# 3DAnimals/3DAnimals

Measured on AMD Instinct MI355X. Metric: train images/sec fwd+bwd @256x256 b16, higher is better.
Workload: dtype f32

## Files before the change

3danimals_amd/_lib.py:

```python
from __future__ import annotations

import ctypes
import os

import torch

_HERE = os.path.dirname(os.path.abspath(__file__))
LIB_PATH = os.environ.get("A3D_LIB") or os.path.join(_HERE, "lib", "liba3d_hip.so")

_c_int, _c_float, _c_size_t, _p = ctypes.c_int, ctypes.c_float, ctypes.c_size_t, ctypes.c_void_p

SIGNATURES = {
    "a3d_version": (_c_int, []),
    "a3d_last_error": (ctypes.c_char_p, []),
    "a3d_bw_probe_fill": (_c_int, [_p, ctypes.c_int64, _p]),
    "a3d_bw_probe_read": (_c_int, [_p, ctypes.c_int64, _p, _p]),
    "a3d_dmtet_scratch_bytes": (_c_size_t, [_c_int, _c_int]),
    "a3d_dmtet_count": (_c_int, [_p, _p, _p, _c_int, _c_int, _p, _p, _p, _c_int, _c_int, _p, _p, _c_int, _p, _c_int, _p]),
    "a3d_dmtet_count_ordered": (_c_int, [_p, _c_int, _c_int, _c_int, _p, _p, _p, _p, _c_int, _p, _c_int, _p]),
    "a3d_dmtet_word_group_slots": (_c_int, []),
    "a3d_dmtet_word_group_bits": (_c_int, []),
    "a3d_dmtet_block_items": (_c_int, []),
    "a3d_dmtet_vertex_scratch_bytes": (_c_size_t, [_c_int]),
    "a3d_dmtet_gather_rows": (_c_int, [_p, _p, ctypes.c_int64, ctypes.c_int64, _c_int, _p, _p]),
# ... 95 lines not shown
    _fields_ = [("size", ctypes.c_uint32), ("lists_stride", ctypes.c_int32), ("prev_rast", _p), ("cover_scratch", _p), ("aa_screen", _p),
                ("aa_count", _p), ("topo_off", _p), ("topo_adj", _p), ("topo_opp", _p), ("normals_v_a", _p), ("normals_v_b", _p),
                ("normals_off", _p), ("normals_adj", _p), ("normals_acc_a", _p), ("normals_a", _p), ("normals_acc_b", _p), ("normals_b", _p),
                ("normals_B_a", ctypes.c_int32), ("normals_B_b", ctypes.c_int32), ("bins", _p), ("bin_cap", ctypes.c_int32), ("bins_clean", ctypes.c_int32),
                ("defer_resolve", ctypes.c_int32), ("reserved", ctypes.c_int32)]


class AaRide(ctypes.Structure):

    _fields_ = [("size", ctypes.c_uint32), ("clip_batch", ctypes.c_int32), ("rast", _p), ("screen", _p), ("tri", _p), ("opp", _p), ("off", _p),
                ("adj", _p), ("V", ctypes.c_int32), ("F", ctypes.c_int32), ("lists_stride", ctypes.c_int32), ("reserved", ctypes.c_int32)]


class CaBuffer(ctypes.Structure):

    _fields_ = [("size", ctypes.c_uint32), ("C", ctypes.c_int32), ("vals", _p), ("bg", _p), ("out", _p), ("g_out", _p), ("g_vals", _p),
                ("bg_batch", ctypes.c_int32), ("reserved", ctypes.c_int32), ("bg_channels", ctypes.c_int32), ("g_stride", ctypes.c_int32),
                ("g_channels", ctypes.c_int32), ("out_channels", ctypes.c_int32), ("vals_rows", ctypes.c_int64)]


class CaShade(ctypes.Structure):

    _fields_ = [("size", ctypes.c_uint32), ("kd_stride", ctypes.c_int32), ("gb", _p), ("par", _p), ("kd", _p), ("clear", _p),
                ("n_clear", ctypes.c_int32), ("two_sided", ctypes.c_int32), ("params", _p), ("shaded_out", _p)]


class ShadeParams(ctypes.Structure):

    _fields_ = [("size", ctypes.c_uint32), ("rot_row_stride", ctypes.c_int32), ("rot", _p), ("view", _p), ("light", _p),
                ("rot_image_stride", ctypes.c_int64), ("view_image_stride", ctypes.c_int64), ("light_image_stride", ctypes.c_int64)]


class EstimateBonesArgs(ctypes.Structure):

    _fields_ = [("size", ctypes.c_uint32), ("N", ctypes.c_int32), ("pos", _p), ("bones", _p), ("nearest", _p), ("ok", _p), ("V", ctypes.c_int32),
                ("n_body", ctypes.c_int32), ("n_leg", ctypes.c_int32), ("body_mode_y_plus", ctypes.c_int32), ("use_y_threshold", ctypes.c_int32),
                ("y_threshold", ctypes.c_float), ("attach", ctypes.c_int32 * 4), ("blend", ctypes.c_float * 17), ("ramp", ctypes.c_float * 9), ("workspace", _p)]


class GbAux(ctypes.Structure):

    _fields_ = [("size", ctypes.c_uint32), ("reserved", ctypes.c_int32), ("tex_out", _p), ("img_out", _p), ("rows", ctypes.c_int64),
                ("pad_to", ctypes.c_int64)]


class DmtetEmitOpts(ctypes.Structure):

    _fields_ = [("size", ctypes.c_uint32), ("Nv", ctypes.c_int32), ("vertex_scratch", _p), ("surf_idx", _p), ("g_sdf_to_clear", _p), ("tri32", _p),
                ("topo_count", _p), ("topo_adj", _p), ("device_counts", _p), ("n_surf", ctypes.c_int32), ("topo_stride", ctypes.c_int32),
                ("use_block_lists", ctypes.c_int32), ("n_edge_blocks_listed", ctypes.c_int32), ("n_tet_blocks_listed", ctypes.c_int32),
                ("surf_bucket", ctypes.c_int32), ("surf_pts", _p)]


class TexDesc(ctypes.Structure):

    _fields_ = [("size", ctypes.c_uint32), ("C", ctypes.c_int32), ("tex_batch", ctypes.c_int32), ("filter", ctypes.c_int32), ("boundary", ctypes.c_int32),
                ("levels", ctypes.c_int32), ("height", ctypes.c_int32 * 16), ("width", ctypes.c_int32 * 16), ("level", _p * 16), ("grad", _p * 16)]


class EnvDesc(ctypes.Structure):

    _fields_ = [("size", ctypes.c_uint32), ("N", ctypes.c_int32), ("roughness", ctypes.c_float), ("costheta_cutoff", ctypes.c_float), ("src", _p),
                ("dst", _p), ("bounds", _p), ("area", _p)]


class BsdfDesc(ctypes.Structure):

    _fields_ = [("size", ctypes.c_uint32), ("op", ctypes.c_int32), ("variant", ctypes.c_int32), ("min_roughness", ctypes.c_float),
                ("ndim", ctypes.c_int32), ("reserved", ctypes.c_int32), ("shape", ctypes.c_int64 * 4), ("seg", ctypes.c_int64), ("in", _p * 6),
                ("stride", ctypes.c_int64 * 24), ("cstride", ctypes.c_int64 * 6), ("out", _p), ("scratch", _p), ("g_out", _p),
                ("g_mode", ctypes.c_int32 * 6), ("seg_div", ctypes.c_int64 * 6), ("g_in", _p * 6), ("g_final", _p * 6)]


BSDF_SIGNATURES = {
    "a3d_bsdf_rows": (ctypes.c_int64, [_p]),
    "a3d_bsdf_fwd": (_c_int, [_p, _p]),
    "a3d_bsdf_bwd": (_c_int, [_p, _p]),
    "a3d_image_loss_fwd": (_c_int, [_p, _p]),
    "a3d_image_loss_bwd": (_c_int, [_p, _p]),
}
BSDF_TILE = 1024
BSDF_MAX_DIMS = 4

ABI_VERSION = 404
_lib = None


class A3DError(RuntimeError):
    pass


def lib():
    global _lib
    if _lib is None:
        if not os.path.exists(LIB_PATH):
            raise A3DError(
                f"{LIB_PATH} is missing: build it with `python 3danimals_amd/csrc/build.py` "
                "(or __graft_entry__.build()).  There is no CPU fallback for the HIP hot path."
            )
        handle = ctypes.CDLL(LIB_PATH)
        for name, (res, args) in list(SIGNATURES.items()) + list(BSDF_SIGNATURES.items()):
            fn = getattr(handle, name)
            fn.restype, fn.argtypes = res, args
        if handle.a3d_version() != ABI_VERSION:
            raise A3DError(f"{LIB_PATH} has ABI version {handle.a3d_version()}, this package binds version {ABI_VERSION}: rebuild it "
                           "with `python 3danimals_amd/csrc/build.py`")
        _lib = handle
    return _lib


class KernelTimer:

    active = None

    def __init__(self):
        self.records = {}

    def __enter__(self):
        KernelTimer.active = self
        return self

    def __exit__(self, *exc):
        KernelTimer.active = None
        return False

    def summary(self):
        torch.cuda.synchronize()
        out = {}
        for name, pairs in self.records.items():
            ms = [a.elapsed_time(b) for a, b in pairs]
            out[name] = (len(ms), sum(ms) / max(len(ms), 1))
        return out


GUARD = int(os.environ.get("A3D_GUARD", "0") or 0)
GUARD_BYTES = 256
_GUARD_BYTE = 0xA5
_guard_live = []
guard_stats = dict(checks=0, buffers_checked=0, allocations=0)


def set_guard(level):
    global GUARD
    import importlib

    prev, GUARD = GUARD, int(level)
    ops = importlib.import_module(__package__ + ".ops")
    ops.torch = GuardedTorch(torch) if GUARD else torch
    if not GUARD:
        _guard_live.clear()
    return prev


def guarded_empty(shape, dtype, device, zero=False, site=""):
    dtype = dtype or torch.get_default_dtype()
    shape = tuple(int(v) for v in shape)
    n = 1
    for v in shape:
        n *= v
    item = torch.empty((), dtype=dtype).element_size()
    nbytes = n * item
    pad = (-nbytes) % 16
    base = torch.empty(GUARD_BYTES + nbytes + pad + GUARD_BYTES, dtype=torch.uint8, device=device)
    base[:GUARD_BYTES] = _GUARD_BYTE
    base[GUARD_BYTES + nbytes:] = _GUARD_BYTE
    t = base[GUARD_BYTES:GUARD_BYTES + nbytes].view(dtype).view(shape)
    if zero:
        t.zero_()
    elif GUARD >= 2 and n:
        if dtype.is_floating_point:
            t.fill_(float("nan"))
        elif dtype == torch.bool:
            t.fill_(True)
        elif item == 1:
            t.fill_(0x7F)
        else:
            t.fill_(0x7F7F7F7F if item >= 4 else 0x7F7F)
    _guard_live.append((base.untyped_storage(), nbytes, f"{dtype} {list(shape)} allocated at {site}"))
    guard_stats["allocations"] += 1
    return t


class GuardedTorch:

# ... 208 lines not shown
```

3danimals_amd/csrc/build.py:

```python
import os
import subprocess
import sys
from concurrent.futures import ThreadPoolExecutor

HERE = os.path.dirname(os.path.abspath(__file__))
PKG = os.path.dirname(HERE)
LIB_DIR = os.path.join(PKG, "lib")
LIB = os.path.join(LIB_DIR, "liba3d_hip.so")
OBJ_DIR = os.path.join(HERE, "build")

SOURCES = {
    "common.hip": [],
    "dmtet.hip": ["-ffp-contract=off"],
    "skin.hip": [],
    "bones.hip": [],
    "normals.hip": ["-ffp-contract=off"],
    "raster.hip": ["-ffp-contract=off"],
    "cover.hip": [],
    "shade.hip": ["-ffp-contract=off"],
    "interp.hip": [],
    "gbuffer.hip": [],
    "segsum.hip": [],
    "losses.hip": [],
    "embed.hip": ["-ffp-contract=off"],
    "gemm.hip": [],
    "antialias.hip": ["-ffp-contract=off"],
    "topology.hip": [],
    "xfm.hip": ["-ffp-contract=off"],
    "texture.hip": ["-ffp-contract=off"],
    "envlight.hip": ["-ffp-contract=off"],
    "bsdf.hip": ["-ffp-contract=off"],
}
COMMON = ["--offload-arch=gfx950", "-O3", "-std=c++17", "-fPIC", "-fhip-fp32-correctly-rounded-divide-sqrt", "-Wall",
          "-Wno-unused-function"]


def _hipcc():
    for c in (os.environ.get("HIPCC"), "/opt/rocm/bin/hipcc", "hipcc"):
        if c and (os.path.isabs(c) and os.path.exists(c) or not os.path.isabs(c)):
            return c
    raise RuntimeError("hipcc not found")


def _stale(target, deps):
    if not os.path.exists(target):
        return True
    t = os.path.getmtime(target)
    return any(os.path.getmtime(d) > t for d in deps)


def build(force=False, verbose=True, profile=False, exp=False):
    assert not (profile and exp)
    lib = os.path.join(LIB_DIR, "liba3d_hip_prof.so") if profile else (os.path.join(LIB_DIR, "liba3d_hip_exp.so") if exp else LIB)
    obj_dir = os.path.join(OBJ_DIR, "prof") if profile else (os.path.join(OBJ_DIR, "exp") if exp else OBJ_DIR)
    os.makedirs(LIB_DIR, exist_ok=True)
    os.makedirs(obj_dir, exist_ok=True)
    hipcc = _hipcc()
    headers = sorted(os.path.join(HERE, f) for f in os.listdir(HERE) if f.endswith(".h")) + [os.path.join(os.path.dirname(PKG), "include", h) for h in ("a3d.h", "a3d_bsdf.h")] + [os.path.abspath(__file__)]
    jobs = []
    objs = []
    for src, extra in SOURCES.items():
        s = os.path.join(HERE, src)
        o = os.path.join(obj_dir, src.replace(".hip", ".o"))
        objs.append(o)
        if force or _stale(o, [s] + headers):
            jobs.append([hipcc, "-x", "hip", "-c", s, "-o", o] + COMMON + extra + (["-DA3D_PROFILE"] if profile else []) + (["-DA3D_EXPERIMENT"] if exp else []))

    def run(cmd):
        if verbose:
            print(" ".join(cmd), flush=True)
        subprocess.check_call(cmd)

    with ThreadPoolExecutor(max_workers=min(8, max(1, len(jobs)))) as ex:
        list(ex.map(run, jobs))
    if force or jobs or _stale(lib, objs):
        run([hipcc, "--offload-arch=gfx950", "-shared", "-fPIC", "-o", lib] + objs)
    return lib


if __name__ == "__main__":
    print(build(force="--force" in sys.argv, profile="--profile" in sys.argv, exp="--exp" in sys.argv))
```

3danimals_amd/csrc/gemm.hip:

```cpp
#include "a3d_common.h"

namespace {

typedef float f32x16 __attribute__((ext_vector_type(16)));
typedef float f32x4 __attribute__((ext_vector_type(4)));

constexpr int GM_N = 256, GM_BK = 32, GM_APAD = GM_BK + 1;

template <int WM, int WN, int BN, int OCC, bool MASK>
__global__ __launch_bounds__(64 * WM * WN, OCC) void gm_nn_kernel(const float* __restrict__ A, const float* __restrict__ B,
                                                                  const float* __restrict__ X, int M, int K, float* __restrict__ C) {
    constexpr int BM = 32 * WM, NT = 64 * WM * WN, TN = BN / WN / 32;
    constexpr int A_F4 = BM * GM_BK / 4 / NT;
    constexpr int B_F4 = GM_BK * BN / 4 / NT;
    static_assert(A_F4 >= 1 && B_F4 >= 1 && BM * GM_BK / 4 % NT == 0 && GM_BK * BN / 4 % NT == 0, "tile / thread count mismatch");
    constexpr int A_ROWS_PER_PASS = NT / 8;
    constexpr int B_ROWS_PER_PASS = NT / (BN / 4);
    __shared__ float As[BM * GM_APAD];
    __shared__ float Bs[GM_BK * BN];
    const int tid = threadIdx.x, lane = tid & 63, wave = tid >> 6, wm = wave / WN, wn = wave - wm * WN;
    const long long m0 = (long long)blockIdx.x * BM;
    const int n0 = blockIdx.y * BN;

    f32x16 acc[TN];
#pragma unroll
    for (int j = 0; j < TN; ++j)
#pragma unroll
        for (int r = 0; r < 16; ++r) acc[j][r] = 0.f;

    static_assert(!MASK || TN == 4, "the masked path keeps the signs of its 64 outputs per lane in one 64-bit word");
    unsigned long long xmask = 0ull;
    const int col0 = n0 + wn * (BN / WN) + (lane & 31);
    const long long mrow = m0 + 32 * wm + 4 * (lane >> 5);
    const float* x_lane = MASK ? X + col0 : nullptr;
    const int a_row = tid >> 3, a_kq = tid & 7, b_row = tid / (BN / 4), b_nq = tid - b_row * (BN / 4);
    const float* a_src = A + (m0 + a_row) * K + 4 * a_kq;
    const float* b_src = B + (long long)b_row * GM_N + n0 + 4 * b_nq;
    f32x4 ra[A_F4], rb[B_F4];
    const f32x4 zero4 = {0.f, 0.f, 0.f, 0.f};
#pragma unroll
    for (int i = 0; i < A_F4; ++i)
        ra[i] = m0 + a_row + A_ROWS_PER_PASS * i < M ? *reinterpret_cast<const f32x4*>(a_src + (long long)A_ROWS_PER_PASS * i * K) : zero4;
#pragma unroll
    for (int i = 0; i < B_F4; ++i) rb[i] = *reinterpret_cast<const f32x4*>(b_src + (long long)B_ROWS_PER_PASS * i * GM_N);

    for (int k0 = 0; k0 < K; k0 += GM_BK) {
        __syncthreads();
#pragma unroll
        for (int i = 0; i < A_F4; ++i) {
            float* d = As + (a_row + A_ROWS_PER_PASS * i) * GM_APAD + 4 * a_kq;
            d[0] = ra[i].x; d[1] = ra[i].y; d[2] = ra[i].z; d[3] = ra[i].w;
        }
#pragma unroll
        for (int i = 0; i < B_F4; ++i) *reinterpret_cast<f32x4*>(Bs + (b_row + B_ROWS_PER_PASS * i) * BN + 4 * b_nq) = rb[i];
        __syncthreads();
        {
            const int kn = k0 + GM_BK < K ? k0 + GM_BK : 0;
            const float* ap = a_src + kn;
            const float* bp = b_src + (long long)kn * GM_N;
#pragma unroll
            for (int i = 0; i < A_F4; ++i)
                ra[i] = m0 + a_row + A_ROWS_PER_PASS * i < M ? *reinterpret_cast<const f32x4*>(ap + (long long)A_ROWS_PER_PASS * i * K) : zero4;
#pragma unroll
            for (int i = 0; i < B_F4; ++i) rb[i] = *reinterpret_cast<const f32x4*>(bp + (long long)B_ROWS_PER_PASS * i * GM_N);
        }
        float xv[MASK ? 8 : 1];
        if (MASK) {
            const int c = (k0 / GM_BK) & 7;
            const float* xb = x_lane + 32 * (c >> 1);
            const long long r0 = mrow + 16 * (c & 1);
#pragma unroll
            for (int dq = 0; dq < 2; ++dq)
#pragma unroll
                for (int sx = 0; sx < 4; ++sx) {
                    const long long rr = r0 + 8 * dq + sx;
                    xv[4 * dq + sx] = xb[(rr < M ? rr : M - 1) * GM_N];
                }
        }
        const float* a_base = As + (32 * wm + (lane & 31)) * GM_APAD + (lane >> 5);
        const float* b_base = Bs + (lane >> 5) * BN + wn * (BN / WN) + (lane & 31);
        float av_n = a_base[0], bv_n[TN];
#pragma unroll
        for (int j = 0; j < TN; ++j) bv_n[j] = b_base[32 * j];
// ... 48 lines not shown
    const int n0 = half * G3_BN;
#pragma unroll
    for (int i = 0; i < 8; ++i) {
        const int f = tid + 1024 * i, k = f >> 5, q = f & 31;
        *reinterpret_cast<f32x4*>(Bs + k * G3_BN + 4 * q) = *reinterpret_cast<const f32x4*>(B + (long long)k * GM_N + n0 + 4 * q);
    }
    __syncthreads();

    const int row = lane & 31, kh = lane >> 5;
    const int n_tiles = (M + 31) >> 5;
    const int stride = nb * G3_WAVES;
    const float* b_lane = Bs + 4 * kh * G3_BN + row;
    for (int t = (wave >> 2) * (nb * 4) + bid * 4 + (wave & 3); t < n_tiles; t += stride) {
        const long long m0 = 32ll * t;
        const long long mr = m0 + row < M ? m0 + row : M - 1;
        const float* a_lane = A + mr * K + 4 * kh;
        f32x16 acc[TN];
#pragma unroll
        for (int j = 0; j < TN; ++j)
#pragma unroll
            for (int r = 0; r < 16; ++r) acc[j][r] = 0.f;
        const long long mrow = m0 + 4 * kh;
        const float* x_wave = MASK ? X + n0 + 4 * row : nullptr;

        f32x4 an[4];
#pragma unroll
        for (int i = 0; i < 4; ++i) an[i] = *reinterpret_cast<const f32x4*>(a_lane + 8 * i);
#pragma unroll 1
        for (int c = 0; c < 8; ++c) {
            f32x4 av[4];
#pragma unroll
            for (int i = 0; i < 4; ++i) av[i] = an[i];
            {
                const int cn = c + 1 < 8 ? c + 1 : 0;
#pragma unroll
                for (int i = 0; i < 4; ++i) an[i] = *reinterpret_cast<const f32x4*>(a_lane + 32 * cn + 8 * i);
            }
            f32x4 xw[MASK ? 2 : 1];
            if (MASK) {
#pragma unroll
                for (int q = 0; q < 2; ++q) {
                    long long rr = m0 + 2 * (2 * c + q) + kh;
                    rr = rr < M ? rr : M - 1;
                    xw[q] = *reinterpret_cast<const f32x4*>(x_wave + rr * GM_N);
                }
            }
            const float* bc = b_lane + (32 * c) * G3_BN;
#pragma unroll
            for (int g = 0; g < 4; ++g)
#pragma unroll
                for (int u = 0; u < 4; ++u) {
                    const float* bp = bc + (8 * g + u) * G3_BN;
#pragma unroll
                    for (int j = 0; j < TN; ++j) acc[j] = __builtin_amdgcn_mfma_f32_32x32x2f32(av[g][u], bp[32 * j], acc[j], 0, 0, 0);
                }
            if (MASK) {
#pragma unroll
                for (int q = 0; q < 2; ++q)
#pragma unroll
                    for (int k4 = 0; k4 < 4; ++k4) {
                        const unsigned long long bal = __ballot(xw[q][k4] > 0.f);
                        if (lane == 0) sign_w[(2 * c + q) * 4 + k4] = bal;
                    }
            }
        }
        if (MASK) __builtin_amdgcn_fence(__ATOMIC_ACQ_REL, "wavefront");
#pragma unroll
        for (int r = 0; r < 16; ++r) {
            const long long m = mrow + (r & 3) + 8 * (r >> 2);
            unsigned long long wv = 0ull;
            if (MASK) wv = sign_w[(2 * kh + ((r & 3) >> 1) + 4 * (r >> 2)) * 4 + (row & 3)] >> ((r & 1) * 32 + (row >> 2));
            if (m < M) {
#pragma unroll
                for (int j = 0; j < TN; ++j) {
                    float v = acc[j][r];
                    if (MASK) v = (wv >> (8 * j)) & 1ull ? v : 0.f;
                    C[m * GM_N + n0 + 32 * j + row] = v;
                }
            }
        }
    }
}

}

extern "C" int a3d_gemm_nn_relumask(const float* A, const float* B, const float* X, int64_t M, int N, int K, float* C, a3d_stream_t stream) {
    A3D_CHECK_ARG(M >= 0 && N == GM_N && K > 0 && K % GM_BK == 0 && M < 0x7fffffffll);
    A3D_CHECK_ARG(X == nullptr || K >= 256);
    if (M == 0) return A3D_OK;
    A3D_CHECK_ARG(A && B && C);
    hipStream_t s = (hipStream_t)stream;
#ifdef A3D_EXPERIMENT
    static const int variant = getenv("A3D_GEMM_VARIANT") ? atoi(getenv("A3D_GEMM_VARIANT")) : 3;
#else
    const int variant = 3;
#endif
    const dim3 block256(256);
    if (variant == 3 && K == 256) {
        static int n_cu_of[64] = {0};
        int dev = 0;
        A3D_HIP(hipGetDevice(&dev));
        A3D_CHECK_ARG(dev >= 0 && dev < 64);
        if (!n_cu_of[dev]) {
            int n = 0;
            A3D_HIP(hipDeviceGetAttribute(&n, hipDeviceAttributeMultiprocessorCount, dev));
            A3D_HIP(hipFuncSetAttribute(reinterpret_cast<const void*>(gm_nn3_kernel<true>), hipFuncAttributeMaxDynamicSharedMemorySize, (256 * G3_BN * 4 + 16 * 64 * 8)));
            A3D_HIP(hipFuncSetAttribute(reinterpret_cast<const void*>(gm_nn3_kernel<false>), hipFuncAttributeMaxDynamicSharedMemorySize, (256 * G3_BN * 4 + 16 * 64 * 8)));
            n_cu_of[dev] = n;
        }
        const int n_cu = n_cu_of[dev];
        const dim3 grid(n_cu & ~1), block(64 * G3_WAVES);
        if (X) hipLaunchKernelGGL(gm_nn3_kernel<true>, grid, block, (256 * G3_BN * 4 + 16 * 64 * 8), s, A, B, X, (int)M, C);
        else hipLaunchKernelGGL(gm_nn3_kernel<false>, grid, block, (256 * G3_BN * 4 + 16 * 64 * 8), s, A, B, X, (int)M, C);
        A3D_LAUNCH_CHECK();
        return A3D_OK;
    }
    if (variant == 1) {
        const dim3 grid(a3d_div_up(M, 64), 1);
        if (X) hipLaunchKernelGGL((gm_nn_kernel<2, 2, 256, 3, true>), grid, block256, 0, s, A, B, X, (int)M, K, C);
        else hipLaunchKernelGGL((gm_nn_kernel<2, 2, 256, 3, false>), grid, block256, 0, s, A, B, X, (int)M, K, C);
    } else {
        const dim3 grid(a3d_div_up(M, 128), 2);
        if (X) hipLaunchKernelGGL((gm_nn_kernel<4, 1, 128, 3, true>), grid, block256, 0, s, A, B, X, (int)M, K, C);
        else hipLaunchKernelGGL((gm_nn_kernel<4, 1, 128, 4, false>), grid, block256, 0, s, A, B, X, (int)M, K, C);
    }
    A3D_LAUNCH_CHECK();
    return A3D_OK;
}
```

3danimals_amd/ops.py:

```python
from __future__ import annotations

import ctypes
import math
import os
from collections import OrderedDict

import torch

from . import _lib
from ._lib import call, f32c, f32h, ptr, require_device, stream


class _IdentityCache:

    def __init__(self, maxsize=8):
        self.maxsize = maxsize
        self.data = OrderedDict()

    @staticmethod
    def key(t):
        return (t.data_ptr(), tuple(t.shape), t.dtype, t._version)

    def get(self, t, make):
        k = self.key(t)
# ... 1582 lines not shown
    def backward(ctx, g_loss, _g_both=None):
        shaded, dino, image_gt, dino_gt, mask_gt, dt0, dt1, valid, both = ctx.saved_tensors
        B, H, W = shaded.shape[:3]
        D = 0 if dino is None else dino.shape[3]
        if g_loss is None:
            return (None,) * 8
        g_shaded = torch.empty_like(shaded)
        ds = dino.stride(2) if D else 0
        g_dino = torch.empty((B, H, W, ds), dtype=torch.float32, device=shaded.device)[..., :D] if D else None
        call("a3d_recon_losses_bwd", ptr(f32h(g_loss)), ptr(shaded), ptr(dino), D, ds, ds, ptr(image_gt), ptr(dino_gt), ptr(mask_gt), ptr(dt0), ptr(dt1),
             dt0.stride(0), ptr(valid), B, H, W, ptr(both), ptr(g_shaded), ptr(g_dino), stream())
        return g_shaded, g_dino, None, None, None, None, None, None


def reconstruction_losses(shaded_nchw, dino_nchw, image_gt, dino_gt, mask_gt, mask_dt, mask_valid, return_mask=False):
    shaded = shaded_nchw.permute(0, 2, 3, 1)
    shaded = shaded if shaded.is_contiguous() else shaded.contiguous()
    dino = None
    if dino_nchw is not None:
        dino = dino_nchw.permute(0, 2, 3, 1)
        H, W, S = dino.shape[1], dino.shape[2], dino.stride(2)
        if not (dino.dtype == torch.float32 and dino.stride(3) == 1 and S >= dino.shape[3] and dino.stride(1) == W * S and dino.stride(0) == H * W * S):
            dino = dino.contiguous()
    loss, both = _ReconLosses.apply(shaded, dino, image_gt, dino_gt, mask_gt, mask_dt[:, 0], mask_dt[:, 1], mask_valid)
    return (loss, both) if return_mask else loss


class _FlowLoss(torch.autograd.Function):
    @staticmethod
    def forward(ctx, flow, flow_gt, both, B, F):
        require_device(flow, flow_gt, both, what="flow_loss")
        N, H, W = flow.shape[:3]
        assert N == B * F and F >= 2 and flow.shape[3] == 2 and flow.stride(3) == 1 and flow.stride(1) == W * flow.stride(2) \
            and flow.stride(0) == H * flow.stride(1), "flow must be the renderer's NHWC buffer (channel slice allowed)"
        flow_gt = f32c(flow_gt)
        assert flow_gt.shape == (B, F - 1, 2, H, W) and both.numel() == N * H * W
        loss = torch.empty((B, F - 1), dtype=torch.float32, device=flow.device)
        scale = torch.empty_like(loss)
        scratch = torch.empty(_lib.lib().a3d_flow_loss_scratch_bytes(B, F, H, W), dtype=torch.uint8, device=flow.device)
        call("a3d_flow_loss_fwd", ptr(flow), flow.stride(2), ptr(flow_gt), ptr(both), B, F, H, W, ptr(scratch), ptr(loss), ptr(scale), stream())
        ctx.save_for_backward(flow, flow_gt, both, scale)
        ctx.dims = (B, F, H, W)
        return loss

    @staticmethod
    def backward(ctx, g_loss):
        flow, flow_gt, both, scale = ctx.saved_tensors
        B, F, H, W = ctx.dims
        g_flow = torch.empty((B * F, H, W, 2), dtype=torch.float32, device=flow.device)
        call("a3d_flow_loss_bwd", ptr(f32h(g_loss)), ptr(scale), ptr(flow), flow.stride(2), ptr(flow_gt), ptr(both), B, F, H, W, ptr(g_flow), stream())
        return g_flow, None, None, None, None


def flow_loss(flow_nchw, flow_gt, both, batch, num_frames):
    return _FlowLoss.apply(flow_nchw.permute(0, 2, 3, 1), flow_gt, both, int(batch), int(num_frames))


class _HarmonicEmbed(torch.autograd.Function):
    @staticmethod
    def forward(ctx, x, freq, symmetrize, ones):
        require_device(x, freq, what="harmonic_embed")
        x, freq = f32c(x), f32c(freq)
        P, n = x.shape[0], freq.shape[0]
        assert x.shape == (P, 3)
        out = torch.empty((P, 3 + 6 * n + int(ones)), dtype=torch.float32, device=x.device)
        call("a3d_harmonic_embed_fwd", ptr(x), ptr(freq), n, int(symmetrize), int(ones), P, ptr(out), stream())
        ctx.save_for_backward(x, freq)
        ctx.cfg = (int(symmetrize), int(ones))
        return out

    @staticmethod
    @torch.autograd.function.once_differentiable
    def backward(ctx, g):
        x, freq = ctx.saved_tensors
        g_x = torch.empty_like(x)
        call("a3d_harmonic_embed_bwd", ptr(f32h(g)), ptr(x), ptr(freq), freq.shape[0], ctx.cfg[0], ctx.cfg[1], x.shape[0], ptr(g_x), stream())
        return g_x, None, None, None


def harmonic_embed(x, freq, symmetrize=False, ones=False):
    return _HarmonicEmbed.apply(x, freq, symmetrize, ones)


def gemm_nn_relumask(a, b, x=None):
    require_device(a, b, what="gemm_nn_relumask")
    a, b = f32c(a), f32c(b)
    M, K = a.shape
    assert b.shape == (K, 256) and K % 32 == 0 and (x is None or (x.shape == (M, 256) and x.is_contiguous() and x.dtype == torch.float32))
    c = torch.empty((M, 256), dtype=torch.float32, device=a.device)
    call("a3d_gemm_nn_relumask", ptr(a), ptr(b), ptr(x), M, 256, K, ptr(c), stream())
    return c


_TEX_FILTERS = {"nearest": 0, "linear": 1, "linear-mipmap-nearest": 2, "linear-mipmap-linear": 3}
_TEX_BOUNDARIES = {"wrap": 0, "clamp": 1, "zero": 2, "cube": 3}
TEX_MAX_LEVELS = 16


def texture_filter_mode(filter_mode, uv_da=None, mip_level_bias=None):
    if filter_mode == "auto":
        return "linear-mipmap-linear" if (uv_da is not None or mip_level_bias is not None) else "linear"
    if filter_mode not in _TEX_FILTERS:
        raise ValueError(f"texture: unknown filter_mode {filter_mode!r}")
    return filter_mode


def texture_mip_sizes(height, width, max_mip_level=None):
    sizes = [(int(height), int(width))]
    top = TEX_MAX_LEVELS - 1 if max_mip_level is None else min(int(max_mip_level), TEX_MAX_LEVELS - 1)
    while len(sizes) - 1 < top:
        h, w = sizes[-1]
        if (h == 1 and w == 1) or (h > 1 and h % 2) or (w > 1 and w % 2):
            break
        sizes.append((max(h // 2, 1), max(w // 2, 1)))
    return sizes


def _tex_hw(t, cube):
    if cube:
        if t.dim() != 5 or t.shape[1] != 6 or t.shape[2] != t.shape[3]:
            raise ValueError(f"texture: a cube level must have shape [Bt, 6, S, S, C], got {list(t.shape)}")
        return t.shape[0], t.shape[2], t.shape[3], t.shape[4]
    if t.dim() != 4:
        raise ValueError(f"texture: a 2-D level must have shape [Bt, H, W, C], got {list(t.shape)}")
    return t.shape[0], t.shape[1], t.shape[2], t.shape[3]


def _tex_desc(levels, C, tex_batch, filt, boundary, grads=None):
    d = _lib.TexDesc(size=ctypes.sizeof(_lib.TexDesc), C=C, tex_batch=tex_batch, filter=filt, boundary=boundary, levels=len(levels))
    cube = boundary == _TEX_BOUNDARIES["cube"]
    for l, t in enumerate(levels):
        d.height[l], d.width[l] = (t.shape[2], t.shape[3]) if cube else (t.shape[1], t.shape[2])
        d.level[l] = t.data_ptr()
        if grads is not None and grads[l] is not None:
            d.grad[l] = grads[l].data_ptr()
    return d


class _TextureMip(torch.autograd.Function):

    @staticmethod
    def forward(ctx, tex, sizes, cube):
        require_device(tex, what="texture_construct_mip")
        tex = f32c(tex)
        Bt, _, _, C = _tex_hw(tex, cube)
        lead = (Bt, 6) if cube else (Bt,)
        levels = [tex] + [torch.empty(lead + (h, w, C), dtype=torch.float32, device=tex.device) for h, w in sizes[1:]]
        call("a3d_texture_mip_fwd", ctypes.byref(_tex_desc(levels, C, Bt, 1, 3 if cube else 1)), stream())
        ctx.shapes, ctx.cube = [tuple(t.shape) for t in levels], cube
        return tuple(levels[1:])

    @staticmethod
    @torch.autograd.function.once_differentiable
    def backward(ctx, *g_levels):
        dev = g_levels[0].device if g_levels[0] is not None else torch.device("cuda", torch.cuda.current_device())
        grads = [torch.zeros(ctx.shapes[0], dtype=torch.float32, device=dev)]
        for shape, g in zip(ctx.shapes[1:], g_levels):
            grads.append(torch.zeros(shape, dtype=torch.float32, device=dev) if g is None else f32c(g).clone())
        C, Bt = ctx.shapes[0][-1], ctx.shapes[0][0]
        call("a3d_texture_mip_bwd", ctypes.byref(_tex_desc(grads, C, Bt, 1, 3 if ctx.cube else 1, grads)), stream())
        return grads[0], None, None


class TextureMip:

    def __init__(self, levels, cube):
        self.levels, self.cube = list(levels), cube


def texture_construct_mip(tex, max_mip_level=None, cube_mode=False):
    Bt, H, W, C = _tex_hw(tex, cube_mode)
    with torch.no_grad():
        levels = _TextureMip.apply(tex.detach(), texture_mip_sizes(H, W, max_mip_level), bool(cube_mode)) if (H, W) != (1, 1) else ()
# ... 450 lines not shown
```

Measured before the change: 1029.

## Add split-bf16 MFMA GEMM path for K=256 relu-mask GEMM

Adds a persistent GEMM kernel that splits fp32 operands into three bf16 parts and accumulates six bf16 MFMA products, emulating fp32 accuracy on matrix cores. It becomes the default for the K=256 relu-mask GEMM and also backs a new NT relu GEMM entry point with optional bias. The goal is to replace the slower fp32 tiled kernel with matrix-core throughput. The cost is extra split arithmetic and a small precision difference, because low-order cross terms are dropped.

```diff
diff --git a/3danimals_amd/_lib.py b/3danimals_amd/_lib.py
--- a/3danimals_amd/_lib.py
+++ b/3danimals_amd/_lib.py
@@ -201,6 +201,11 @@
 BSDF_TILE = 1024
 BSDF_MAX_DIMS = 4
 
+GEMM_SIGNATURES = {
+    "a3d_gemm_nn_relumask_mode": (_c_int, [_p, _p, _p, ctypes.c_int64, _c_int, _c_int, _c_int, _p, _p]),
+    "a3d_gemm_nt_relu": (_c_int, [_p, _p, _p, ctypes.c_int64, _c_int, _c_int, _p, _p]),
+}
+
 ABI_VERSION = 404
 _lib = None
 
@@ -218,7 +223,7 @@
                 "(or __graft_entry__.build()).  There is no CPU fallback for the HIP hot path."
             )
         handle = ctypes.CDLL(LIB_PATH)
-        for name, (res, args) in list(SIGNATURES.items()) + list(BSDF_SIGNATURES.items()):
+        for name, (res, args) in list(SIGNATURES.items()) + list(BSDF_SIGNATURES.items()) + list(GEMM_SIGNATURES.items()):
             fn = getattr(handle, name)
             fn.restype, fn.argtypes = res, args
         if handle.a3d_version() != ABI_VERSION:
diff --git a/3danimals_amd/csrc/build.py b/3danimals_amd/csrc/build.py
--- a/3danimals_amd/csrc/build.py
+++ b/3danimals_amd/csrc/build.py
@@ -56,7 +56,7 @@
     os.makedirs(LIB_DIR, exist_ok=True)
     os.makedirs(obj_dir, exist_ok=True)
     hipcc = _hipcc()
-    headers = sorted(os.path.join(HERE, f) for f in os.listdir(HERE) if f.endswith(".h")) + [os.path.join(os.path.dirname(PKG), "include", h) for h in ("a3d.h", "a3d_bsdf.h")] + [os.path.abspath(__file__)]
+    headers = sorted(os.path.join(HERE, f) for f in os.listdir(HERE) if f.endswith(".h")) + [os.path.join(os.path.dirname(PKG), "include", h) for h in ("a3d.h", "a3d_bsdf.h", "a3d_gemm.h")] + [os.path.abspath(__file__)]
     jobs = []
     objs = []
     for src, extra in SOURCES.items():
diff --git a/3danimals_amd/csrc/gemm.hip b/3danimals_amd/csrc/gemm.hip
--- a/3danimals_amd/csrc/gemm.hip
+++ b/3danimals_amd/csrc/gemm.hip
@@ -1,4 +1,5 @@
 #include "a3d_common.h"
+#include "../../include/a3d_gemm.h"
 
 namespace {
 
@@ -213,14 +214,191 @@
     }
 }
 
-}
-
-extern "C" int a3d_gemm_nn_relumask(const float* A, const float* B, const float* X, int64_t M, int N, int K, float* C, a3d_stream_t stream) {
+
+typedef __bf16 bf16x8 __attribute__((ext_vector_type(8)));
+
+constexpr int GM_SPLIT_DEFAULT = 1;
+constexpr int G6_BN = 64, G6_WAVES = 16, G6_LDS = 3 * 32 * G6_BN * 16;
+
+__device__ __forceinline__ void gm_split3(const f32x4 lo, const f32x4 hi, bf16x8& p0, bf16x8& p1, bf16x8& p2) {
+#pragma unroll
+    for (int j = 0; j < 8; ++j) {
+        const float a = j < 4 ? lo[j & 3] : hi[j & 3];
+        const __bf16 q0 = (__bf16)a;
+        const float r1 = a - (float)q0;
+        const __bf16 q1 = (__bf16)r1;
+        const float r2 = r1 - (float)q1;
+        p0[j] = q0; p1[j] = q1; p2[j] = (__bf16)r2;
+    }
+}
+
+template <int MODE>
+__global__ __launch_bounds__(64 * G6_WAVES, 1) void gm_split_kernel(const float* __restrict__ A, const float* __restrict__ B,
+                                                                    const float* __restrict__ X ,
+                                                                    int M, float* __restrict__ C) {
+    constexpr int K = 256;
+    extern __shared__ __attribute__((aligned(16))) unsigned char g6_smem[];
+    bf16x8* Bs = reinterpret_cast<bf16x8*>(g6_smem);
+    const int tid = threadIdx.x, lane = tid & 63, wave = tid >> 6;
+    const int bx = blockIdx.x, quarter = (bx >> 3) & 3, grp = (bx & 7) + 8 * (bx >> 5), ng = gridDim.x >> 2;
+    const int n0 = quarter * G6_BN;
+#pragma unroll
+    for (int i = 0; i < 2; ++i) {
+        const int f = tid + 1024 * i, col = f & 63, kg = f >> 6;
+        f32x4 lo, hi;
+        if (MODE == 2) {
+            const float* w = B + (long long)(n0 + col) * K + 8 * kg;
+            lo = *reinterpret_cast<const f32x4*>(w);
+            hi = *reinterpret_cast<const f32x4*>(w + 4);
+        } else {
+            const float* w = B + (long long)(8 * kg) * GM_N + n0 + col;
+#pragma unroll
+            for (int j = 0; j < 4; ++j) { lo[j] = w[j * GM_N]; hi[j] = w[(4 + j) * GM_N]; }
+        }
+        bf16x8 p0, p1, p2;
+        gm_split3(lo, hi, p0, p1, p2);
+        Bs[(0 * 32 + kg) * G6_BN + col] = p0;
+        Bs[(1 * 32 + kg) * G6_BN + col] = p1;
+        Bs[(2 * 32 + kg) * G6_BN + col] = p2;
+    }
+    __syncthreads();
+
+    const int row = lane & 31, h = lane >> 5;
+    const int n_tiles = (M + 31) >> 5;
+    const int stride = ng * G6_WAVES;
+    const bf16x8* b_lane = Bs + h * G6_BN + row;
+    int t = (wave >> 2) * (ng * 4) + grp * 4 + (wave & 3);
+    if (t >= n_tiles) return;
+    f32x4 an[8];
+    {
+        const long long mr = 32ll * t + row < M ? 32ll * t + row : M - 1;
+        const float* ap = A + mr * K + 8 * h;
+#pragma unroll
+        for (int s = 0; s < 4; ++s) {
+            an[2 * s] = *reinterpret_cast<const f32x4*>(ap + 16 * s);
+            an[2 * s + 1] = *reinterpret_cast<const f32x4*>(ap + 16 * s + 4);
+        }
+    }
+    for (; t < n_tiles; t += stride) {
+        const long long m = 32ll * t + row;
+        const long long mr = m < M ? m : M - 1;
+        const int tn = t + stride < n_tiles ? t + stride : t;
+        const long long mrn = 32ll * tn + row < M ? 32ll * tn + row : M - 1;
+        const float* a_lane = A + mr * K + 8 * h;
+        const float* a_next = A + mrn * K + 8 * h;
+        const float* x_lane = MODE == 1 ? X + mr * GM_N + n0 + 4 * h : nullptr;
+        f32x16 acc[2];
+#pragma unroll
+        for (int r = 0; r < 16; ++r) { acc[0][r] = 0.f; acc[1][r] = 0.f; }
+        unsigned xbits = 0u;
+#pragma unroll 1
+        for (int c = 0; c < 4; ++c) {
+            f32x4 av[8];
+#pragma unroll
+            for (int i = 0; i < 8; ++i) av[i] = an[i];
+            {
+                const float* ap = c < 3 ? a_lane + 64 * (c + 1) : a_next;
+#pragma unroll
+                for (int s = 0; s < 4; ++s) {
+                    an[2 * s] = *reinterpret_cast<const f32x4*>(ap + 16 * s);
+                    an[2 * s + 1] = *reinterpret_cast<const f32x4*>(ap + 16 * s + 4);
+                }
+            }
+            f32x4 xw[MODE == 1 ? 2 : 1];
+            if (MODE == 1) {
+#pragma unroll
+                for (int q = 0; q < 2; ++q) xw[q] = *reinterpret_cast<const f32x4*>(x_lane + 32 * (c >> 1) + 8 * (2 * (c & 1) + q));
+            }
+            const bf16x8* bc = b_lane + (8 * c) * G6_BN;
+#pragma unroll
+            for (int s = 0; s < 4; ++s) {
+                bf16x8 a0, a1, a2;
+                gm_split3(av[2 * s], av[2 * s + 1], a0, a1, a2);
+                const bf16x8* bp = bc + (2 * s) * G6_BN;
+                bf16x8 b0[2], b1[2], b2[2];
+#pragma unroll
+                for (int j = 0; j < 2; ++j) {
+                    b0[j] = bp[32 * j];
+                    b1[j] = bp[32 * G6_BN + 32 * j];
+                    b2[j] = bp[64 * G6_BN + 32 * j];
+                }
+#pragma unroll
+                for (int j = 0; j < 2; ++j) acc[j] = __builtin_amdgcn_mfma_f32_32x32x16_bf16(b2[j], a0, acc[j], 0, 0, 0);
+#pragma unroll
+                for (int j = 0; j < 2; ++j) acc[j] = __builtin_amdgcn_mfma_f32_32x32x16_bf16(b1[j], a1, acc[j], 0, 0, 0);
+#pragma unroll
+                for (int j = 0; j < 2; ++j) acc[j] = __builtin_amdgcn_mfma_f32_32x32x16_bf16(b0[j], a2, acc[j], 0, 0, 0);
+#pragma unroll
+                for (int j = 0; j < 2; ++j) acc[j] = __builtin_amdgcn_mfma_f32_32x32x16_bf16(b1[j], a0, acc[j], 0, 0, 0);
+#pragma unroll
+                for (int j = 0; j < 2; ++j) acc[j] = __builtin_amdgcn_mfma_f32_32x32x16_bf16(b0[j], a1, acc[j], 0, 0, 0);
+#pragma unroll
+                for (int j = 0; j < 2; ++j) acc[j] = __builtin_amdgcn_mfma_f32_32x32x16_bf16(b0[j], a0, acc[j], 0, 0, 0);
+            }
+            if (MODE == 1) {
+#pragma unroll
+                for (int q = 0; q < 2; ++q)
+#pragma unroll
+                    for (int e = 0; e < 4; ++e) xbits |= (unsigned)(xw[q][e] > 0.f) << (16 * (c >> 1) + 4 * (2 * (c & 1) + q) + e);
+            }
+        }
+        if (m < M) {
+            float* c_lane = C + m * GM_N + n0 + 4 * h;
+#pragma unroll
+            for (int j = 0; j < 2; ++j)
+#pragma unroll
+                for (int q = 0; q < 4; ++q) {
+                    f32x4 v;
+#pragma unroll
+                    for (int e = 0; e < 4; ++e) v[e] = acc[j][4 * q + e];
+                    if (MODE == 1) {
+#pragma unroll
+                        for (int e = 0; e < 4; ++e) v[e] = (xbits >> (16 * j + 4 * q + e)) & 1u ? v[e] : 0.f;
+                    }
+                    if (MODE == 2) {
+                        if (X) {
+                            const f32x4 bias = *reinterpret_cast<const f32x4*>(X + n0 + 4 * h + 32 * j + 8 * q);
+#pragma unroll
+                            for (int e = 0; e < 4; ++e) v[e] += bias[e];
+                        }
+#pragma unroll
+                        for (int e = 0; e < 4; ++e) v[e] = v[e] < 0.f ? 0.f : v[e];
+                    }
+                    *reinterpret_cast<f32x4*>(c_lane + 32 * j + 8 * q) = v;
+                }
+        }
+    }
+}
+
+template <int MODE>
+int gm_split_launch(const float* A, const float* B, const float* X, int64_t M, float* C, hipStream_t s) {
+    static int n_cu_of[64] = {0};
+    int dev = 0;
+    A3D_HIP(hipGetDevice(&dev));
+    A3D_CHECK_ARG(dev >= 0 && dev < 64);
+    if (!n_cu_of[dev]) {
+        int n = 0;
+        A3D_HIP(hipDeviceGetAttribute(&n, hipDeviceAttributeMultiprocessorCount, dev));
+        A3D_HIP(hipFuncSetAttribute(reinterpret_cast<const void*>(gm_split_kernel<MODE>), hipFuncAttributeMaxDynamicSharedMemorySize, G6_LDS));
+        n_cu_of[dev] = n;
+    }
+    const int n_cu = n_cu_of[dev];
+    const dim3 grid(n_cu >= 32 ? n_cu & ~31 : 32), block(64 * G6_WAVES);
+    hipLaunchKernelGGL((gm_split_kernel<MODE>), grid, block, G6_LDS, s, A, B, X, (int)M, C);
+    A3D_LAUNCH_CHECK();
+    return A3D_OK;
+}
+
+}
+
+static int gm_nn_dispatch(const float* A, const float* B, const float* X, int64_t M, int N, int K, int mode, float* C, a3d_stream_t stream) {
     A3D_CHECK_ARG(M >= 0 && N == GM_N && K > 0 && K % GM_BK == 0 && M < 0x7fffffffll);
     A3D_CHECK_ARG(X == nullptr || K >= 256);
+    A3D_CHECK_ARG(mode == 0 || (mode == 1 && K == 256));
     if (M == 0) return A3D_OK;
     A3D_CHECK_ARG(A && B && C);
     hipStream_t s = (hipStream_t)stream;
+    if (mode == 1) return X ? gm_split_launch<1>(A, B, X, M, C, s) : gm_split_launch<0>(A, B, X, M, C, s);
 #ifdef A3D_EXPERIMENT
     static const int variant = getenv("A3D_GEMM_VARIANT") ? atoi(getenv("A3D_GEMM_VARIANT")) : 3;
 #else
@@ -258,3 +436,19 @@
     A3D_LAUNCH_CHECK();
     return A3D_OK;
 }
+
+extern "C" int a3d_gemm_nn_relumask(const float* A, const float* B, const float* X, int64_t M, int N, int K, float* C, a3d_stream_t stream) {
+    return gm_nn_dispatch(A, B, X, M, N, K, K == 256 ? GM_SPLIT_DEFAULT : 0, C, stream);
+}
+
+extern "C" int a3d_gemm_nn_relumask_mode(const float* A, const float* B, const float* X, int64_t M, int N, int K, int mode, float* C,
+                                         a3d_stream_t stream) {
+    return gm_nn_dispatch(A, B, X, M, N, K, mode, C, stream);
+}
+
+extern "C" int a3d_gemm_nt_relu(const float* A, const float* W, const float* bias, int64_t M, int N, int K, float* C, a3d_stream_t stream) {
+    A3D_CHECK_ARG(M >= 0 && N == GM_N && K == 256 && M < 0x7fffffffll);
+    if (M == 0) return A3D_OK;
+    A3D_CHECK_ARG(A && W && C);
+    return gm_split_launch<2>(A, W, bias, M, C, (hipStream_t)stream);
+}
diff --git a/3danimals_amd/ops.py b/3danimals_amd/ops.py
--- a/3danimals_amd/ops.py
+++ b/3danimals_amd/ops.py
@@ -1688,13 +1688,29 @@
     return _HarmonicEmbed.apply(x, freq, symmetrize, ones)
 
 
-def gemm_nn_relumask(a, b, x=None):
+GEMM_MODES = {"fp32": 0, "split": 1}
+
+
+def gemm_nn_relumask(a, b, x=None, mode=None):
     require_device(a, b, what="gemm_nn_relumask")
     a, b = f32c(a), f32c(b)
     M, K = a.shape
     assert b.shape == (K, 256) and K % 32 == 0 and (x is None or (x.shape == (M, 256) and x.is_contiguous() and x.dtype == torch.float32))
     c = torch.empty((M, 256), dtype=torch.float32, device=a.device)
-    call("a3d_gemm_nn_relumask", ptr(a), ptr(b), ptr(x), M, 256, K, ptr(c), stream())
+    if mode is None:
+        call("a3d_gemm_nn_relumask", ptr(a), ptr(b), ptr(x), M, 256, K, ptr(c), stream())
+    else:
+        call("a3d_gemm_nn_relumask_mode", ptr(a), ptr(b), ptr(x), M, 256, K, GEMM_MODES[mode], ptr(c), stream())
+    return c
+
+
+def gemm_nt_relu(a, w, bias=None):
+    require_device(a, w, what="gemm_nt_relu")
+    a, w = f32c(a), f32c(w)
+    M = a.shape[0]
+    assert a.shape == (M, 256) and w.shape == (256, 256) and (bias is None or (bias.shape == (256,) and bias.is_contiguous() and bias.dtype == torch.float32))
+    c = torch.empty((M, 256), dtype=torch.float32, device=a.device)
+    call("a3d_gemm_nt_relu", ptr(a), ptr(w), ptr(bias), M, 256, 256, ptr(c), stream())
     return c
 
 
diff --git a/include/a3d_gemm.h b/include/a3d_gemm.h
--- /dev/null
+++ b/include/a3d_gemm.h
@@ -0,0 +1,17 @@
+#ifndef A3D_GEMM_H
+#define A3D_GEMM_H
+#include "a3d.h"
+
+#ifdef __cplusplus
+extern "C" {
+#endif
+
+int a3d_gemm_nn_relumask_mode(const float* A, const float* B, const float* X, int64_t M, int N, int K, int mode, float* C,
+                              a3d_stream_t stream);
+
+int a3d_gemm_nt_relu(const float* A, const float* W, const float* bias, int64_t M, int N, int K, float* C, a3d_stream_t stream);
+
+#ifdef __cplusplus
+}
+#endif
+#endif
```

After: 1068 (median of 4 runs). 3.8% higher.
